# lifuguan/IGGT_official

Measured on NVIDIA H100. Metric: views/sec (518^2, V=8), higher is better.
Workload: dtype fp16

## Files before the change

### iggt_official_b200/csrc/gemm.cuh

```cuda
#pragma once
#include "ptx.cuh"
#include "launch.cuh"

namespace iggt {

enum GemmEpi : int {
  EPI_STORE16 = 0,
  EPI_RESID32 = 1,
  EPI_QKV = 2,
  EPI_STORE32 = 3,
  EPI_QKV_GATHER = 4,
};
__host__ __device__ constexpr bool epi_is_qkv(int e) { return e == EPI_QKV || e == EPI_QKV_GATHER; }

struct GemmParams {
  int M, N, K;
  int num_m_tiles, num_n_tiles, num_k_blocks;
  const float* bias;
  const float* gamma;
  int act;
  int qk_norm;
  int C;
  const float* qn_w; const float* qn_b; const float* kn_w; const float* kn_b;
  const float* rope_cos; const float* rope_sin;
  const int* pos_yx;
  int T;
  const void* addend; int add_rows; int add_ld;
  int conv_taps;
  int conv_C;
  int H, W, NB;
  int tiles_x, tiles_y;
  const void* resid;
  const void* resid2;
  int act_post;
  int round_out16;
  const CUtensorMap* gather_maps;
  int n_gather;
  int gather_col0;
  int gather_rows;
  int stream_k;
};

constexpr int GEMM_BM = 128;
constexpr int GEMM_BK = 64;
constexpr int GEMM_THREADS = 384;
constexpr int CONV_TW = 16;
constexpr int CONV_TH = 8;

template <int BN>
struct GemmSmem {
  static constexpr int A_BYTES = GEMM_BM * GEMM_BK * 2;
  static constexpr int B_BYTES = BN * GEMM_BK * 2;
  static constexpr int STAGE_BYTES = A_BYTES + B_BYTES;
  static constexpr int STG_BYTES = 16384;
  static constexpr int ACC_LD = BN + 8;
  static constexpr int ACC_BYTES = GEMM_BM * ACC_LD * 4;
  static constexpr int STAGES = BN == 128 ? 3 : 6;
  static constexpr int VEC_BYTES = BN * 4 + (BN * 4 > 1024 ? BN * 4 : 1024);
  static constexpr int TOTAL = STAGES * STAGE_BYTES + ACC_BYTES + 2 * STG_BYTES + 256  + VEC_BYTES;
};

template <bool BF16>
__device__ __forceinline__ float cvt16_to_f32(uint16_t h) {
  if constexpr (BF16) return __uint_as_float(static_cast<uint32_t>(h) << 16);
  else return __half2float(__ushort_as_half(h));
}
template <bool BF16>
__device__ __forceinline__ float round16(float x) {
  if constexpr (BF16) return __bfloat162float(__float2bfloat16_rn(x));
  else return __half2float(__float2half_rn(x));
}

__device__ __forceinline__ float apply_act(float x, int act) {
  if (act == 1) return gelu_fast(x);
  if (act == 2) return relu_nan(x);
  if (act == 3) return x > 0.0f ? x : 0.01f * x;
  return x;
}

struct WorkIter {
  int pos, end, step, kb_per_tile, num_tiles;
  bool sk;
  __device__ WorkIter(const GemmParams& p, int worker, int workers) {
    kb_per_tile = p.num_k_blocks;
    num_tiles = p.num_m_tiles * p.num_n_tiles;
    sk = p.stream_k != 0;
    if (sk) {
      const long total = static_cast<long>(num_tiles) * kb_per_tile;
      const long per = (total + workers - 1) / workers;
      const long b = static_cast<long>(worker) * per;
      pos = static_cast<int>(b < total ? b : total);
      end = static_cast<int>(b + per < total ? b + per : total);
      step = 0;
    } else {
      pos = worker; end = num_tiles; step = workers;
    }
  }
  __device__ bool next(int& tile, int& kb0, int& kb1) {
    if (pos >= end) return false;
    if (sk) {
      tile = pos / kb_per_tile;
      kb0 = pos - tile * kb_per_tile;
      const int room = end - pos;
      kb1 = kb0 + room < kb_per_tile ? kb0 + room : kb_per_tile;
      pos += kb1 - kb0;
    } else {
      tile = pos; kb0 = 0; kb1 = kb_per_tile; pos += step;
    }
    return true;
  }
};

template <int BN, int EPI, bool BF16, bool CONV>
__global__ void __launch_bounds__(GEMM_THREADS, 1)
gemm_wgmma_kernel(const __grid_constant__ CUtensorMap tmA, const __grid_constant__ CUtensorMap tmB,
                  const __grid_constant__ CUtensorMap tmC, const GemmParams p) {
  using SM = GemmSmem<BN>;
  constexpr int STAGES = SM::STAGES;
  constexpr int G = 2;
  extern __shared__ __align__(1024) uint8_t smem[];
  if ((smem_u32(smem) & 1023u) != 0) __trap();
  uint8_t* smem_a = smem;
  uint8_t* smem_b = smem + STAGES * SM::A_BYTES;
  float* acc_tile = reinterpret_cast<float*>(smem + STAGES * SM::STAGE_BYTES);
  uint8_t* staging = smem + STAGES * SM::STAGE_BYTES + SM::ACC_BYTES;
  uint64_t* bars = reinterpret_cast<uint64_t*>(staging + 2 * SM::STG_BYTES);
  uint64_t* full_bar = bars;
  uint64_t* empty_bar = bars + STAGES;
  float* epi_vec = reinterpret_cast<float*>(reinterpret_cast<uint8_t*>(bars) + 256);

  const int warp = threadIdx.x >> 5;
  const int lane = threadIdx.x & 31;
  const int worker = static_cast<int>(blockIdx.x);
  const int workers = static_cast<int>(gridDim.x);

  if (warp == 0 && lane == 0) {
    tma_prefetch_desc(&tmA);
    tma_prefetch_desc(&tmB);
    tma_prefetch_desc(&tmC);
  }
  if (warp == 1 && lane == 0) {
    for (int i = 0; i < STAGES; ++i) {
      mbar_init(&full_bar[i], 1);
      mbar_init(&empty_bar[i], G);
    }
    fence_barrier_init();
  }
  __syncthreads();
  griddep_wait();
  griddep_launch();

  if (warp < 4) {
    if (warp == 0 && lane == 0) {
      int stage = 0;
      uint32_t phase = 0;
      WorkIter work(p, worker, workers);
      int tile, kb0, kb1;
      while (work.next(tile, kb0, kb1)) {
        const int mt = tile / p.num_n_tiles;
        const int nt = tile % p.num_n_tiles;
        int img = 0, y0 = 0, x0 = 0;
        if constexpr (CONV) {
          const int per_img = p.tiles_x * p.tiles_y;
          img = mt / per_img;
          const int r = mt % per_img;
          y0 = (r / p.tiles_x) * CONV_TH;
          x0 = (r % p.tiles_x) * CONV_TW;
        }
        for (int kb = kb0; kb < kb1; ++kb) {
          mbar_wait(&empty_bar[stage], phase ^ 1);
          int dy = 0, dx = 0, c0 = 0;
          if constexpr (CONV) {
            const int cblocks = p.conv_C / GEMM_BK;
            const int tap = kb / cblocks;
            c0 = (kb % cblocks) * GEMM_BK;
            if (p.conv_taps == 9) { dy = tap / 3 - 1; dx = tap % 3 - 1; }
          }
          mbar_expect_tx(&full_bar[stage], SM::STAGE_BYTES);
          if constexpr (CONV) tma_load_4d(smem_a + stage * SM::A_BYTES, &tmA, &full_bar[stage], c0, x0 + dx, y0 + dy, img);
          else tma_load_2d(smem_a + stage * SM::A_BYTES, &tmA, &full_bar[stage], kb * GEMM_BK, mt * GEMM_BM);
          tma_load_2d(smem_b + stage * SM::B_BYTES, &tmB, &full_bar[stage], kb * GEMM_BK, nt * BN);
          if (++stage == STAGES) { stage = 0; phase ^= 1; }
        }
      }
    }
  } else {
    const int grp = (warp - 4) >> 2;
    const int ew = (warp - 4) & 3;
    const int row = ew * 32 + lane;
    const bool leader = (ew == 0 && lane == 0);
    constexpr int NBUF = 2 / G;
    uint8_t* const stg_grp = staging + grp * NBUF * SM::STG_BYTES;
    const uint32_t bar_id = 1 + grp;
    const int gtid = ew * 32 + lane;
    float* const vb = epi_vec;
    float* const vg = vb + BN;
    float* const vn = vb + BN;
    if constexpr (epi_is_qkv(EPI)) {
      if (p.qk_norm) {
        for (int i = gtid; i < 64; i += 128) {
          vn[i] = p.qn_w[i]; vn[64 + i] = p.qn_b[i]; vn[128 + i] = p.kn_w[i]; vn[192 + i] = p.kn_b[i];
        }
      }
    }
    int stage = 0;
    uint32_t phase = 0;
    uint32_t store_count = 0;
    WorkIter work(p, worker, workers);
    int tile, kb0, kb1;
    while (work.next(tile, kb0, kb1)) {
      const int mt = tile / p.num_n_tiles;
      const int nt = tile % p.num_n_tiles;
      const int n0 = nt * BN;
      float acc[BN / 2];
#pragma unroll
      for (int i = 0; i < BN / 2; ++i) acc[i] = 0.f;
      int prev_stage = -1;
      for (int kb = kb0; kb < kb1; ++kb) {
        mbar_wait(&full_bar[stage], phase);
        const uint32_t a_addr = smem_u32(smem_a + stage * SM::A_BYTES) + grp * (64 * 128);
        const uint32_t b_addr = smem_u32(smem_b + stage * SM::B_BYTES);
        wgmma_fence();
#pragma unroll
        for (int k = 0; k < GEMM_BK / 16; ++k) {
          const uint64_t da = make_desc_sw128(a_addr + k * 32, 1024);
          const uint64_t db = make_desc_sw128(b_addr + k * 32, 1024);
          if constexpr (BN == 128) wgmma_m64n128k16_ss<BF16>(acc, da, db, (kb != kb0 || k != 0) ? 1u : 0u);
          else wgmma_m64n64k16_ss<BF16>(acc, da, db, (kb != kb0 || k != 0) ? 1u : 0u);
        }
        wgmma_commit();
        wgmma_wait<1>();
        if (prev_stage >= 0 && gtid == 0) mbar_arrive(&empty_bar[prev_stage]);
        prev_stage = stage;
        if (++stage == STAGES) { stage = 0; phase ^= 1; }
      }
      wgmma_wait<0>();
      reg_fence(acc);
      if (prev_stage >= 0 && gtid == 0) mbar_arrive(&empty_bar[prev_stage]);

      int img = 0, y0 = 0, x0 = 0;
      long grow;
      if constexpr (CONV) {
        const int per_img = p.tiles_x * p.tiles_y;
        img = mt / per_img;
        const int r = mt % per_img;
        y0 = (r / p.tiles_x) * CONV_TH;
        x0 = (r % p.tiles_x) * CONV_TW;
        const int yy = y0 + row / CONV_TW, xx = x0 + row % CONV_TW;
        grow = (yy < p.H && xx < p.W && img < p.NB) ? ((long)img * p.H + yy) * p.W + xx : -1;
      } else {
        grow = (long)mt * GEMM_BM + row;
        if (grow >= p.M) grow = -1;
      }
      named_bar_sync(3, 128 * G);
      {
        const int r0 = grp * 64 + ew * 16 + (lane >> 2);
        float* const d0 = acc_tile + r0 * SM::ACC_LD + 2 * (lane & 3);
#pragma unroll
        for (int j = 0; j < BN / 8; ++j) {
          *reinterpret_cast<float2*>(d0 + 8 * j) = make_float2(acc[4 * j], acc[4 * j + 1]);
          *reinterpret_cast<float2*>(d0 + 8 * SM::ACC_LD + 8 * j) = make_float2(acc[4 * j + 2], acc[4 * j + 3]);
        }
      }
      for (int i = grp * 128 + gtid; i < BN; i += 128 * G) {
        const int col = n0 + i;
        vb[i] = (p.bias && col < p.N && kb0 == 0) ? __ldg(p.bias + col) : 0.f;
        if constexpr (EPI == EPI_RESID32) vg[i] = (p.gamma && col < p.N) ? __ldg(p.gamma + col) : 1.f;
      }
      named_bar_sync(3, 128 * G);
      const float* const t_row = acc_tile + row * SM::ACC_LD;

      if constexpr (EPI == EPI_STORE16 || epi_is_qkv(EPI)) {
        const int nvalid = min(BN / 64, (p.N - n0 + 63) / 64);
#pragma unroll 1
        for (int c64 = grp; c64 < nvalid; c64 += G) {
          const int col0 = n0 + c64 * 64;
          uint8_t* stg = stg_grp + (store_count % NBUF) * SM::STG_BYTES;
          if (leader) tma_store_wait_read<NBUF - 1>();
          named_bar_sync(bar_id, 128);
          float v[64];
#pragma unroll
          for (int i = 0; i < 64; i += 4) {
            const float4 a = *reinterpret_cast<const float4*>(t_row + c64 * 64 + i);
            v[i] = a.x; v[i + 1] = a.y; v[i + 2] = a.z; v[i + 3] = a.w;
          }
          {
#pragma unroll
            for (int i = 0; i < 64; i += 4) {
              const float4 b = *reinterpret_cast<const float4*>(vb + c64 * 64 + i);
              const float2 lo = fadd2(make_float2(v[i], v[i + 1]), make_float2(b.x, b.y));
              const float2 hi = fadd2(make_float2(v[i + 2], v[i + 3]), make_float2(b.z, b.w));
              v[i] = lo.x; v[i + 1] = lo.y; v[i + 2] = hi.x; v[i + 3] = hi.y;
            }
          }
          if constexpr (epi_is_qkv(EPI)) {
            if (p.qk_norm && col0 < 2 * p.C) {
              const bool is_k = col0 >= p.C;
              const float* nw = vn + (is_k ? 128 : 0);
              const float* nb = nw + 64;
              float s = 0.f;
#pragma unroll
              for (int i = 0; i < 64; ++i) { v[i] = round16<BF16>(v[i]); s += v[i]; }
              const float mean = s * (1.0f / 64.0f);
              float q = 0.f;
#pragma unroll
              for (int i = 0; i < 64; ++i) { const float d = v[i] - mean; q += d * d; }
              const float rstd = rsqrtf(q * (1.0f / 64.0f) + 1e-5f);
#pragma unroll
              for (int i = 0; i < 64; ++i) v[i] = (v[i] - mean) * rstd * nw[i] + nb[i];
              const int t = (grow >= 0) ? static_cast<int>(grow % p.T) : 0;
              const int py = __ldg(p.pos_yx + 2 * t), px = __ldg(p.pos_yx + 2 * t + 1);
#pragma unroll
              for (int h = 0; h < 2; ++h) {
                const int ps = h == 0 ? py : px;
                const float* cs = p.rope_cos + ps * 16;
                const float* sn = p.rope_sin + ps * 16;
#pragma unroll
                for (int i = 0; i < 16; ++i) {
                  const float c = __ldg(cs + i), s_ = __ldg(sn + i);
                  const float a = v[h * 32 + i], b = v[h * 32 + 16 + i];
                  v[h * 32 + i] = a * c - b * s_;
                  v[h * 32 + 16 + i] = b * c + a * s_;
                }
              }
            }
          } else {
            if (p.act == 1) {
#pragma unroll
              for (int i = 0; i < 64; i += 2) {
                const float2 g = gelu_fast2(make_float2(round16<BF16>(v[i]), round16<BF16>(v[i + 1])));
                v[i] = g.x; v[i + 1] = g.y;
              }
            } else if (p.act == 5) {
#pragma unroll
              for (int i = 0; i < 64; i += 2) {
                const float2 g = gelu_erfc2(make_float2(round16<BF16>(v[i]), round16<BF16>(v[i + 1])));
                v[i] = g.x; v[i + 1] = g.y;
              }
            } else if (p.act) {
#pragma unroll
              for (int i = 0; i < 64; ++i) v[i] = apply_act(v[i], p.act);
            }
            if (p.addend && grow >= 0) {
              const uint16_t* ad = reinterpret_cast<const uint16_t*>(p.addend) +
                                   (grow % p.add_rows) * (long)p.add_ld + col0;
#pragma unroll
              for (int i = 0; i < 64; i += 8) {
                if (col0 + i < p.N) {
                  const uint4 u = __ldg(reinterpret_cast<const uint4*>(ad + i));
                  const uint32_t w[4] = {u.x, u.y, u.z, u.w};
#pragma unroll
                  for (int j = 0; j < 4; ++j) {
                    v[i + 2 * j] += cvt16_to_f32<BF16>(static_cast<uint16_t>(w[j] & 0xFFFF));
                    v[i + 2 * j + 1] += cvt16_to_f32<BF16>(static_cast<uint16_t>(w[j] >> 16));
                  }
                }
              }
            }
            if constexpr (CONV) {
#pragma unroll
              for (int rr = 0; rr < 2; ++rr) {
                const void* rp = rr == 0 ? p.resid : p.resid2;
                if (rp && grow >= 0) {
                  const uint16_t* ad = reinterpret_cast<const uint16_t*>(rp) + grow * (long)p.N + col0;
#pragma unroll
                  for (int i = 0; i < 64; i += 8) {
                    if (col0 + i < p.N) {
                      const uint4 u = __ldg(reinterpret_cast<const uint4*>(ad + i));
                      const uint32_t w[4] = {u.x, u.y, u.z, u.w};
#pragma unroll
                      for (int j = 0; j < 4; ++j) {
                        v[i + 2 * j] += cvt16_to_f32<BF16>(static_cast<uint16_t>(w[j] & 0xFFFF));
                        v[i + 2 * j + 1] += cvt16_to_f32<BF16>(static_cast<uint16_t>(w[j] >> 16));
                      }
                    }
                  }
                }
              }
              if (p.act_post) {
#pragma unroll
                for (int i = 0; i < 64; ++i) v[i] = apply_act(v[i], p.act_post);
              }
            }
          }
          bool later_scene = false;
          if constexpr (EPI == EPI_QKV_GATHER) {
            if (p.n_gather > 0 && col0 >= p.gather_col0 && grow >= 0)
              later_scene = grow / p.gather_rows != (static_cast<long>(mt) * GEMM_BM) / p.gather_rows;
          }
#pragma unroll
          for (int c = 0; c < 8; ++c) {
            uint4 u;
            u.x = pack16x2<BF16>(v[c * 8 + 0], v[c * 8 + 1]);
            u.y = pack16x2<BF16>(v[c * 8 + 2], v[c * 8 + 3]);
            u.z = pack16x2<BF16>(v[c * 8 + 4], v[c * 8 + 5]);
            u.w = pack16x2<BF16>(v[c * 8 + 6], v[c * 8 + 7]);
            *reinterpret_cast<uint4*>(stg + row * 128 + ((c ^ (row & 7)) << 4)) = u;
            if constexpr (EPI == EPI_QKV_GATHER) {
              if (later_scene) {
                void* const* ptrs = reinterpret_cast<void* const*>(p.gather_maps + p.n_gather);
                const long* lds = reinterpret_cast<const long*>(ptrs + p.n_gather);
                const long scene = grow / p.gather_rows, rr = grow - scene * p.gather_rows;
                const long off = scene * __ldg(lds + 1) + rr * __ldg(lds) + (col0 - p.gather_col0) + c * 8;
                for (int r = 0; r < p.n_gather; ++r)
                  *reinterpret_cast<uint4*>(reinterpret_cast<uint16_t*>(ptrs[r]) + off) = u;
              }
            }
          }
          if constexpr (EPI == EPI_QKV_GATHER) {
            if (later_scene) __threadfence_system();
          }
          fence_proxy_async_smem();
          named_bar_sync(bar_id, 128);
          if (leader) {
            if constexpr (CONV) tma_store_4d(&tmC, stg, col0, x0, y0, img);
            else tma_store_2d(&tmC, stg, col0, mt * GEMM_BM);
            if constexpr (EPI == EPI_QKV_GATHER) {
              if (p.n_gather > 0 && col0 >= p.gather_col0) {
                const int row0 = mt * GEMM_BM, scene = row0 / p.gather_rows, r0 = row0 - scene * p.gather_rows;
                for (int r = 0; r < p.n_gather; ++r)
                  tma_store_3d(&p.gather_maps[r], stg, col0 - p.gather_col0, r0, scene);
              }
            }
            tma_store_commit();
          }
          ++store_count;
        }
      } else {
        const int nvalid = min(BN / 32, (p.N - n0 + 31) / 32);
#pragma unroll 1
        for (int c32 = grp; c32 < nvalid; c32 += G) {
          const int col0 = n0 + c32 * 32;
          uint8_t* stg = stg_grp + (store_count % NBUF) * SM::STG_BYTES;
          if (leader) tma_store_wait_read<NBUF - 1>();
          named_bar_sync(bar_id, 128);
          float v[32];
#pragma unroll
          for (int i = 0; i < 32; i += 4) {
            const float4 a = *reinterpret_cast<const float4*>(t_row + c32 * 32 + i);
            v[i] = a.x; v[i + 1] = a.y; v[i + 2] = a.z; v[i + 3] = a.w;
          }
#pragma unroll
          for (int i = 0; i < 32; i += 4) {
            const float4 b = *reinterpret_cast<const float4*>(vb + c32 * 32 + i);
            float2 lo = fadd2(make_float2(v[i], v[i + 1]), make_float2(b.x, b.y));
            float2 hi = fadd2(make_float2(v[i + 2], v[i + 3]), make_float2(b.z, b.w));
            if constexpr (EPI == EPI_RESID32) {
              if (p.round_out16 && !p.stream_k) {
                lo.x = round16<BF16>(lo.x); lo.y = round16<BF16>(lo.y);
                hi.x = round16<BF16>(hi.x); hi.y = round16<BF16>(hi.y);
              }
              const float4 g = *reinterpret_cast<const float4*>(vg + c32 * 32 + i);
              lo = fmul2(lo, make_float2(g.x, g.y));
              hi = fmul2(hi, make_float2(g.z, g.w));
            }
            v[i] = lo.x; v[i + 1] = lo.y; v[i + 2] = hi.x; v[i + 3] = hi.y;
          }
          if constexpr (EPI == EPI_STORE32) {
            if (p.act) {
#pragma unroll
              for (int i = 0; i < 32; ++i) v[i] = apply_act(v[i], p.act);
            }
          }
#pragma unroll
          for (int c = 0; c < 8; ++c) {
            float4 u = make_float4(v[c * 4], v[c * 4 + 1], v[c * 4 + 2], v[c * 4 + 3]);
            *reinterpret_cast<float4*>(stg + row * 128 + ((c ^ (row & 7)) << 4)) = u;
          }
          fence_proxy_async_smem();
          named_bar_sync(bar_id, 128);
          if (leader) {
            if constexpr (EPI == EPI_RESID32) tma_reduce_add_2d(&tmC, stg, col0, mt * GEMM_BM);
            else tma_store_2d(&tmC, stg, col0, mt * GEMM_BM);
            tma_store_commit();
          }
          ++store_count;
        }
      }
    }
    if (leader) {
      tma_store_wait_all<0>();
      if constexpr (EPI == EPI_QKV_GATHER) {
        if (p.n_gather > 0) __threadfence_system();
      }
    }
  }
}

}
```

### iggt_official_b200/csrc/ptx.cuh

```cuda
#pragma once
#include <cuda.h>
#include <cuda_fp16.h>
#include <cuda_bf16.h>
#include <cuda_runtime.h>
#include <stdint.h>

namespace iggt {

__device__ __forceinline__ uint32_t smem_u32(const void* p) {
  return static_cast<uint32_t>(__cvta_generic_to_shared(p));
}
__device__ __forceinline__ uint32_t lane_id() { return threadIdx.x & 31; }

__device__ __forceinline__ bool elect_one() {
  uint32_t pred = 0;
  asm volatile(
      "{\n\t.reg .pred P;\n\t"
      "elect.sync _|P, 0xffffffff;\n\t"
      "selp.b32 %0, 1, 0, P;\n\t}\n"
      : "=r"(pred));
  return pred != 0;
}

__device__ __forceinline__ void mbar_init(uint64_t* bar, uint32_t count) {
  asm volatile("mbarrier.init.shared::cta.b64 [%0], %1;" ::"r"(smem_u32(bar)), "r"(count));
}
__device__ __forceinline__ void fence_barrier_init() {
  asm volatile("fence.mbarrier_init.release.cluster;" ::: "memory");
}
__device__ __forceinline__ void mbar_expect_tx(uint64_t* bar, uint32_t bytes) {
  asm volatile("mbarrier.arrive.expect_tx.shared::cta.b64 _, [%0], %1;" ::"r"(smem_u32(bar)),
               "r"(bytes)
               : "memory");
}
__device__ __forceinline__ void mbar_arrive(uint64_t* bar) {
  asm volatile("mbarrier.arrive.shared::cta.b64 _, [%0];" ::"r"(smem_u32(bar)) : "memory");
}
__device__ __forceinline__ bool mbar_try_wait(uint64_t* bar, uint32_t parity) {
  uint32_t ok;
  asm volatile(
      "{\n\t.reg .pred P;\n\t"
      "mbarrier.try_wait.parity.shared::cta.b64 P, [%1], %2;\n\t"
      "selp.b32 %0, 1, 0, P;\n\t}\n"
      : "=r"(ok)
      : "r"(smem_u32(bar)), "r"(parity)
      : "memory");
  return ok != 0;
}
__device__ __forceinline__ void mbar_wait(uint64_t* bar, uint32_t parity) {
  while (!mbar_try_wait(bar, parity)) {
  }
}

__device__ __forceinline__ void fence_proxy_async_smem() {
  asm volatile("fence.proxy.async.shared::cta;" ::: "memory");
}
__device__ __forceinline__ void named_bar_sync(uint32_t id, uint32_t nthreads) {
  asm volatile("bar.sync %0, %1;" ::"r"(id), "r"(nthreads) : "memory");
}

__device__ __forceinline__ void tma_prefetch_desc(const CUtensorMap* m) {
  asm volatile("prefetch.tensormap [%0];" ::"l"(reinterpret_cast<uint64_t>(m)) : "memory");
}
__device__ __forceinline__ void tma_load_2d(void* smem, const CUtensorMap* m, uint64_t* bar,
                                            int32_t c0, int32_t c1) {
  asm volatile(
      "cp.async.bulk.tensor.2d.shared::cluster.global.mbarrier::complete_tx::bytes"
      " [%0], [%1, {%3, %4}], [%2];" ::"r"(smem_u32(smem)),
      "l"(reinterpret_cast<uint64_t>(m)), "r"(smem_u32(bar)), "r"(c0), "r"(c1)
      : "memory");
}
__device__ __forceinline__ void tma_load_3d(void* smem, const CUtensorMap* m, uint64_t* bar,
                                            int32_t c0, int32_t c1, int32_t c2) {
  asm volatile(
      "cp.async.bulk.tensor.3d.shared::cluster.global.mbarrier::complete_tx::bytes"
      " [%0], [%1, {%3, %4, %5}], [%2];" ::"r"(smem_u32(smem)),
      "l"(reinterpret_cast<uint64_t>(m)), "r"(smem_u32(bar)), "r"(c0), "r"(c1), "r"(c2)
      : "memory");
}
__device__ __forceinline__ void tma_load_4d(void* smem, const CUtensorMap* m, uint64_t* bar,
                                            int32_t c0, int32_t c1, int32_t c2, int32_t c3) {
  asm volatile(
      "cp.async.bulk.tensor.4d.shared::cluster.global.mbarrier::complete_tx::bytes"
      " [%0], [%1, {%3, %4, %5, %6}], [%2];" ::"r"(smem_u32(smem)),
      "l"(reinterpret_cast<uint64_t>(m)), "r"(smem_u32(bar)), "r"(c0), "r"(c1), "r"(c2), "r"(c3)
      : "memory");
}
__device__ __forceinline__ void tma_bulk_load_1d(void* smem, const void* gptr, uint32_t bytes, uint64_t* bar) {
  asm volatile("cp.async.bulk.shared::cluster.global.mbarrier::complete_tx::bytes [%0], [%1], %2, [%3];" ::"r"(
                   smem_u32(smem)),
               "l"(reinterpret_cast<uint64_t>(gptr)), "r"(bytes), "r"(smem_u32(bar))
               : "memory");
}
__device__ __forceinline__ void tma_store_2d(const CUtensorMap* m, const void* smem, int32_t c0,
                                             int32_t c1) {
  asm volatile("cp.async.bulk.tensor.2d.global.shared::cta.bulk_group [%0, {%2, %3}], [%1];" ::"l"(
                   reinterpret_cast<uint64_t>(m)),
               "r"(smem_u32(smem)), "r"(c0), "r"(c1)
               : "memory");
}
__device__ __forceinline__ void tma_store_3d(const CUtensorMap* m, const void* smem, int32_t c0, int32_t c1, int32_t c2) {
  asm volatile("cp.async.bulk.tensor.3d.global.shared::cta.bulk_group [%0, {%2, %3, %4}], [%1];" ::"l"(
                   reinterpret_cast<uint64_t>(m)),
               "r"(smem_u32(smem)), "r"(c0), "r"(c1), "r"(c2)
               : "memory");
}
__device__ __forceinline__ void tma_store_4d(const CUtensorMap* m, const void* smem, int32_t c0,
                                             int32_t c1, int32_t c2, int32_t c3) {
  asm volatile(
      "cp.async.bulk.tensor.4d.global.shared::cta.bulk_group [%0, {%2, %3, %4, %5}], [%1];" ::"l"(
          reinterpret_cast<uint64_t>(m)),
      "r"(smem_u32(smem)), "r"(c0), "r"(c1), "r"(c2), "r"(c3)
      : "memory");
}
__device__ __forceinline__ void tma_reduce_add_2d(const CUtensorMap* m, const void* smem,
                                                  int32_t c0, int32_t c1) {
  asm volatile(
      "cp.reduce.async.bulk.tensor.2d.global.shared::cta.add.tile.bulk_group [%0, {%2, %3}], [%1];" ::
          "l"(reinterpret_cast<uint64_t>(m)),
      "r"(smem_u32(smem)), "r"(c0), "r"(c1)
      : "memory");
}
__device__ __forceinline__ void tma_store_commit() {
  asm volatile("cp.async.bulk.commit_group;" ::: "memory");
}
template <int N>
__device__ __forceinline__ void tma_store_wait_read() {
  asm volatile("cp.async.bulk.wait_group.read %0;" ::"n"(N) : "memory");
}
template <int N>
__device__ __forceinline__ void tma_store_wait_all() {
  asm volatile("cp.async.bulk.wait_group %0;" ::"n"(N) : "memory");
}

__device__ __forceinline__ void wgmma_fence() { asm volatile("wgmma.fence.sync.aligned;" ::: "memory"); }
__device__ __forceinline__ void wgmma_commit() { asm volatile("wgmma.commit_group.sync.aligned;" ::: "memory"); }
template <int N>
__device__ __forceinline__ void wgmma_wait() {
  asm volatile("wgmma.wait_group.sync.aligned %0;" ::"n"(N) : "memory");
}
template <int R>
__device__ __forceinline__ void reg_fence(float (&d)[R]) {
#pragma unroll
  for (int i = 0; i < R; ++i) asm volatile("" : "+f"(d[i])::"memory");
}

#define IGGT_D8(o) "+f"(d[o]), "+f"(d[o + 1]), "+f"(d[o + 2]), "+f"(d[o + 3]), "+f"(d[o + 4]), "+f"(d[o + 5]), \
                   "+f"(d[o + 6]), "+f"(d[o + 7])
#define IGGT_WGMMA_SS_32(T)                                                                                     \
  asm volatile("{\n\t.reg .pred p;\n\tsetp.ne.b32 p, %18, 0;\n\t"                                               \
               "wgmma.mma_async.sync.aligned.m64n32k16.f32." T "." T " {%0, %1, %2, %3, %4, %5, %6, %7, %8, %9, %10, %11, %12, %13, %14, %15}, %16, %17, p, 1, 1, 0, 0;\n\t}\n" \
               : IGGT_D8(0), IGGT_D8(8)                                                                                          \
               : "l"(a_desc), "l"(b_desc), "r"(accumulate))
template <bool BF16>
__device__ __forceinline__ void wgmma_m64n32k16_ss(float (&d)[16], uint64_t a_desc, uint64_t b_desc, uint32_t accumulate) {
  if constexpr (BF16) IGGT_WGMMA_SS_32("bf16");
  else IGGT_WGMMA_SS_32("f16");
}
#define IGGT_WGMMA_SS_64(T)                                                                                     \
  asm volatile("{\n\t.reg .pred p;\n\tsetp.ne.b32 p, %34, 0;\n\t"                                               \
               "wgmma.mma_async.sync.aligned.m64n64k16.f32." T "." T " {%0, %1, %2, %3, %4, %5, %6, %7, %8, %9, %10, %11, %12, %13, %14, %15, %16, %17, %18, %19, %20, %21, %22, %23, %24, %25, %26, %27, %28, %29, %30, %31}, %32, %33, p, 1, 1, 0, 0;\n\t}\n" \
               : IGGT_D8(0), IGGT_D8(8), IGGT_D8(16), IGGT_D8(24)                                                                                          \
               : "l"(a_desc), "l"(b_desc), "r"(accumulate))
template <bool BF16>
__device__ __forceinline__ void wgmma_m64n64k16_ss(float (&d)[32], uint64_t a_desc, uint64_t b_desc, uint32_t accumulate) {
  if constexpr (BF16) IGGT_WGMMA_SS_64("bf16");
  else IGGT_WGMMA_SS_64("f16");
}
#define IGGT_WGMMA_SS_128(T)                                                                                     \
  asm volatile("{\n\t.reg .pred p;\n\tsetp.ne.b32 p, %66, 0;\n\t"                                               \
               "wgmma.mma_async.sync.aligned.m64n128k16.f32." T "." T " {%0, %1, %2, %3, %4, %5, %6, %7, %8, %9, %10, %11, %12, %13, %14, %15, %16, %17, %18, %19, %20, %21, %22, %23, %24, %25, %26, %27, %28, %29, %30, %31, %32, %33, %34, %35, %36, %37, %38, %39, %40, %41, %42, %43, %44, %45, %46, %47, %48, %49, %50, %51, %52, %53, %54, %55, %56, %57, %58, %59, %60, %61, %62, %63}, %64, %65, p, 1, 1, 0, 0;\n\t}\n" \
               : IGGT_D8(0), IGGT_D8(8), IGGT_D8(16), IGGT_D8(24), IGGT_D8(32), IGGT_D8(40), IGGT_D8(48), IGGT_D8(56)                                                                                          \
               : "l"(a_desc), "l"(b_desc), "r"(accumulate))
template <bool BF16>
__device__ __forceinline__ void wgmma_m64n128k16_ss(float (&d)[64], uint64_t a_desc, uint64_t b_desc, uint32_t accumulate) {
  if constexpr (BF16) IGGT_WGMMA_SS_128("bf16");
  else IGGT_WGMMA_SS_128("f16");
}
#define IGGT_WGMMA_RS_TB_64(T)                                                                                   \
  asm volatile("{\n\t.reg .pred p;\n\tsetp.ne.b32 p, %37, 0;\n\t"                                               \
               "wgmma.mma_async.sync.aligned.m64n64k16.f32." T "." T " {%0, %1, %2, %3, %4, %5, %6, %7, %8, %9, %10, %11, %12, %13, %14, %15, %16, %17, %18, %19, %20, %21, %22, %23, %24, %25, %26, %27, %28, %29, %30, %31}, {%32, %33, %34, %35}, %36, p, 1, 1, 1;\n\t}\n" \
               : IGGT_D8(0), IGGT_D8(8), IGGT_D8(16), IGGT_D8(24)                                                                                          \
               : "r"(a[0]), "r"(a[1]), "r"(a[2]), "r"(a[3]), "l"(b_desc), "r"(accumulate))
template <bool BF16>
__device__ __forceinline__ void wgmma_m64n64k16_rs_tb(float (&d)[32], const uint32_t (&a)[4], uint64_t b_desc,
                                                      uint32_t accumulate) {
  if constexpr (BF16) IGGT_WGMMA_RS_TB_64("bf16");
  else IGGT_WGMMA_RS_TB_64("f16");
}

__device__ __forceinline__ uint64_t make_desc_sw128(uint32_t smem_addr, uint32_t sbo_bytes) {
  uint64_t d = 0;
  d |= static_cast<uint64_t>((smem_addr & 0x3FFFF) >> 4);
  d |= static_cast<uint64_t>(1) << 16;
  d |= static_cast<uint64_t>((sbo_bytes >> 4) & 0x3FFF) << 32;
  d |= static_cast<uint64_t>(1) << 62;
  return d;
}

__device__ __forceinline__ uint32_t pack_f16x2(float a, float b) {
  __half2 h = __floats2half2_rn(a, b);
  return *reinterpret_cast<uint32_t*>(&h);
}
__device__ __forceinline__ uint32_t pack_bf16x2(float a, float b) {
  __nv_bfloat162 h = __floats2bfloat162_rn(a, b);
  return *reinterpret_cast<uint32_t*>(&h);
}
template <bool BF16>
__device__ __forceinline__ uint32_t pack16x2(float a, float b) {
  if constexpr (BF16) return pack_bf16x2(a, b);
  else return pack_f16x2(a, b);
}
__device__ __forceinline__ float relu_nan(float x) {
  float y;
  asm("max.NaN.f32 %0, %1, 0f00000000;" : "=f"(y) : "f"(x));
  return y;
}
__device__ __forceinline__ float gelu_erf(float x) {
  return 0.5f * x * (1.0f + erff(x * 0.70710678118654752440f));
}
__device__ __forceinline__ float ex2_approx(float x) {
  float y;
  asm("ex2.approx.ftz.f32 %0, %1;" : "=f"(y) : "f"(x));
  return y;
}
__device__ __forceinline__ float2 ffma2(float2 a, float2 b, float2 c) {
  return make_float2(__fmaf_rn(a.x, b.x, c.x), __fmaf_rn(a.y, b.y, c.y));
}
__device__ __forceinline__ float2 fadd2(float2 a, float2 b) {
  return make_float2(__fadd_rn(a.x, b.x), __fadd_rn(a.y, b.y));
}
__device__ __forceinline__ float2 fmul2(float2 a, float2 b) {
  return make_float2(__fmul_rn(a.x, b.x), __fmul_rn(a.y, b.y));
}
__device__ __forceinline__ float gelu_fast(float x) {
  const float z = fabsf(x) * 0.70710678118654752440f;
  const float t = __fdividef(1.0f, fmaf(0.3275911f, z, 1.0f));
  float poly = fmaf(t, 1.061405429f, -1.453152027f);
  poly = fmaf(poly, t, 1.421413741f);
  poly = fmaf(poly, t, -0.284496736f);
  poly = fmaf(poly, t, 0.254829592f);
  poly *= t;
  const float e = ex2_approx(-z * z * 1.4426950408889634f);
  const float erf_abs = fmaf(-poly, e, 1.0f);
  const float hx = 0.5f * x;
  return fmaf(hx, copysignf(erf_abs, x), hx);
}

__device__ __forceinline__ float2 gelu_fast2(float2 x) {
  const float2 ax = make_float2(fabsf(x.x), fabsf(x.y));
  const float2 z = fmul2(ax, make_float2(0.70710678118654752440f, 0.70710678118654752440f));
  const float2 den = ffma2(make_float2(0.3275911f, 0.3275911f), z, make_float2(1.0f, 1.0f));
  const float2 t = make_float2(__fdividef(1.0f, den.x), __fdividef(1.0f, den.y));
  float2 poly = ffma2(t, make_float2(1.061405429f, 1.061405429f), make_float2(-1.453152027f, -1.453152027f));
  poly = ffma2(poly, t, make_float2(1.421413741f, 1.421413741f));
  poly = ffma2(poly, t, make_float2(-0.284496736f, -0.284496736f));
  poly = ffma2(poly, t, make_float2(0.254829592f, 0.254829592f));
  poly = fmul2(poly, t);
  const float2 nz = make_float2(-z.x, -z.y);
  const float2 arg = fmul2(fmul2(nz, z), make_float2(1.4426950408889634f, 1.4426950408889634f));
  const float2 e = make_float2(ex2_approx(arg.x), ex2_approx(arg.y));
  const float2 erf_abs = ffma2(make_float2(-poly.x, -poly.y), e, make_float2(1.0f, 1.0f));
  const float2 hx = fmul2(make_float2(0.5f, 0.5f), x);
  return ffma2(hx, make_float2(copysignf(erf_abs.x, x.x), copysignf(erf_abs.y, x.y)), hx);
}


__device__ __forceinline__ float2 gelu_erfc2(float2 x) {
  const float2 hx = fmul2(x, make_float2(0.5f, 0.5f));
  const float2 na = make_float2(__uint_as_float(__float_as_uint(hx.x) | 0x80000000u),
                                __uint_as_float(__float_as_uint(hx.y) | 0x80000000u));
  float2 z = fmul2(na, make_float2(-1.4142135623730951f, -1.4142135623730951f));
  z.x = fminf(z.x, 4.3f);
  z.y = fminf(z.y, 4.3f);
  float2 q = ffma2(make_float2(-1.5555357094854116e-05f, -1.5555357094854116e-05f), z,
                   make_float2(0.0004183394485153258f, 0.0004183394485153258f));
  q = ffma2(q, z, make_float2(-0.0048510609194636345f, -0.0048510609194636345f));
  q = ffma2(q, z, make_float2(0.03291909396648407f, 0.03291909396648407f));
  q = ffma2(q, z, make_float2(-0.1511300802230835f, -0.1511300802230835f));
  q = ffma2(q, z, make_float2(-0.9178327322006226f, -0.9178327322006226f));
  q = ffma2(q, z, make_float2(-1.6279296875f, -1.6279296875f));
  const float2 pz = fmul2(q, z);
  const float2 e = make_float2(ex2_approx(pz.x), ex2_approx(pz.y));
  const float2 s = ffma2(na, make_float2(-1.0f, -1.0f), hx);
  return ffma2(na, e, s);
}

}
```

Baseline: 59.69.

## Ping-pong consumer warpgroups across tiles with register reallocation

Before, the two consumer warpgroups each took half of every 128-row tile. Now each warpgroup handles the whole 128-row tile (two m64 wgmma accumulators) and the two groups alternate tiles. Named barriers order the MMA phases and the epilogue phases, so one group's epilogue overlaps the other group's MMA. setmaxnreg moves registers from the producer warps to the consumers to hold the doubled accumulator. The cost is more register pressure, a shared accumulator tile and staging buffer that are now serialized, and more complex ring and phase bookkeeping.

```diff
diff --git a/iggt_official_b200/csrc/gemm.cuh b/iggt_official_b200/csrc/gemm.cuh
--- a/iggt_official_b200/csrc/gemm.cuh
+++ b/iggt_official_b200/csrc/gemm.cuh
@@ -117,7 +117,7 @@
                   const __grid_constant__ CUtensorMap tmC, const GemmParams p) {
   using SM = GemmSmem<BN>;
   constexpr int STAGES = SM::STAGES;
-  constexpr int G = 2;
+  constexpr uint32_t BAR_MMA_DONE = 3, BAR_EPI_DONE = 5;
   extern __shared__ __align__(1024) uint8_t smem[];
   if ((smem_u32(smem) & 1023u) != 0) __trap();
   uint8_t* smem_a = smem;
@@ -142,7 +142,7 @@
   if (warp == 1 && lane == 0) {
     for (int i = 0; i < STAGES; ++i) {
       mbar_init(&full_bar[i], 1);
-      mbar_init(&empty_bar[i], G);
+      mbar_init(&empty_bar[i], 1);
     }
     fence_barrier_init();
   }
@@ -151,6 +151,7 @@
   griddep_launch();
 
   if (warp < 4) {
+    reg_dealloc<40>();
     if (warp == 0 && lane == 0) {
       int stage = 0;
       uint32_t phase = 0;
@@ -185,48 +186,64 @@
       }
     }
   } else {
-    const int grp = (warp - 4) >> 2;
+    reg_alloc<232>();
+    const int wg = (warp - 4) >> 2;
     const int ew = (warp - 4) & 3;
     const int row = ew * 32 + lane;
     const bool leader = (ew == 0 && lane == 0);
-    constexpr int NBUF = 2 / G;
-    uint8_t* const stg_grp = staging + grp * NBUF * SM::STG_BYTES;
-    const uint32_t bar_id = 1 + grp;
+    constexpr int NBUF = 2;
+    const uint32_t bar_id = 1 + wg;
     const int gtid = ew * 32 + lane;
     float* const vb = epi_vec;
     float* const vg = vb + BN;
     float* const vn = vb + BN;
     if constexpr (epi_is_qkv(EPI)) {
-      if (p.qk_norm) {
+      if (p.qk_norm && wg == 0) {
         for (int i = gtid; i < 64; i += 128) {
           vn[i] = p.qn_w[i]; vn[64 + i] = p.qn_b[i]; vn[128 + i] = p.kn_w[i]; vn[192 + i] = p.kn_b[i];
         }
       }
     }
-    int stage = 0;
-    uint32_t phase = 0;
     uint32_t store_count = 0;
     WorkIter work(p, worker, workers);
-    int tile, kb0, kb1;
-    while (work.next(tile, kb0, kb1)) {
+    int tile, kb0, kb1, ntile, nkb0, nkb1;
+    bool more = work.next(ntile, nkb0, nkb1);
+    uint32_t ring = 0;
+    int seg_len = 0;
+    for (int seg = 0; more; ++seg) {
+      ring += seg_len;
+      tile = ntile; kb0 = nkb0; kb1 = nkb1;
+      seg_len = kb1 - kb0;
+      more = work.next(ntile, nkb0, nkb1);
+      if ((seg & 1) != wg) continue;
       const int mt = tile / p.num_n_tiles;
       const int nt = tile % p.num_n_tiles;
       const int n0 = nt * BN;
-      float acc[BN / 2];
-#pragma unroll
-      for (int i = 0; i < BN / 2; ++i) acc[i] = 0.f;
+      if (seg > 0) named_bar_sync(BAR_MMA_DONE + (wg ^ 1), 256);
+      int stage = static_cast<int>(ring % STAGES);
+      uint32_t phase = (ring / STAGES) & 1;
+      float acc[2][BN / 2];
+#pragma unroll
+      for (int h = 0; h < 2; ++h) {
+#pragma unroll
+        for (int i = 0; i < BN / 2; ++i) acc[h][i] = 0.f;
+      }
       int prev_stage = -1;
       for (int kb = kb0; kb < kb1; ++kb) {
         mbar_wait(&full_bar[stage], phase);
-        const uint32_t a_addr = smem_u32(smem_a + stage * SM::A_BYTES) + grp * (64 * 128);
+        const uint32_t a_addr = smem_u32(smem_a + stage * SM::A_BYTES);
         const uint32_t b_addr = smem_u32(smem_b + stage * SM::B_BYTES);
         wgmma_fence();
 #pragma unroll
         for (int k = 0; k < GEMM_BK / 16; ++k) {
-          const uint64_t da = make_desc_sw128(a_addr + k * 32, 1024);
           const uint64_t db = make_desc_sw128(b_addr + k * 32, 1024);
-          if constexpr (BN == 128) wgmma_m64n128k16_ss<BF16>(acc, da, db, (kb != kb0 || k != 0) ? 1u : 0u);
-          else wgmma_m64n64k16_ss<BF16>(acc, da, db, (kb != kb0 || k != 0) ? 1u : 0u);
+          const uint32_t accumulate = (kb != kb0 || k != 0) ? 1u : 0u;
+#pragma unroll
+          for (int h = 0; h < 2; ++h) {
+            const uint64_t da = make_desc_sw128(a_addr + h * (64 * 128) + k * 32, 1024);
+            if constexpr (BN == 128) wgmma_m64n128k16_ss<BF16>(acc[h], da, db, accumulate);
+            else wgmma_m64n64k16_ss<BF16>(acc[h], da, db, accumulate);
+          }
         }
         wgmma_commit();
         wgmma_wait<1>();
@@ -234,8 +251,10 @@
         prev_stage = stage;
         if (++stage == STAGES) { stage = 0; phase ^= 1; }
       }
+      if (more) named_bar_arrive(BAR_MMA_DONE + wg, 256);
       wgmma_wait<0>();
-      reg_fence(acc);
+      reg_fence(acc[0]);
+      reg_fence(acc[1]);
       if (prev_stage >= 0 && gtid == 0) mbar_arrive(&empty_bar[prev_stage]);
 
       int img = 0, y0 = 0, x0 = 0;
@@ -252,30 +271,31 @@
         grow = (long)mt * GEMM_BM + row;
         if (grow >= p.M) grow = -1;
       }
-      named_bar_sync(3, 128 * G);
-      {
-        const int r0 = grp * 64 + ew * 16 + (lane >> 2);
+      if (seg > 0) named_bar_sync(BAR_EPI_DONE + (wg ^ 1), 256);
+#pragma unroll
+      for (int h = 0; h < 2; ++h) {
+        const int r0 = h * 64 + ew * 16 + (lane >> 2);
         float* const d0 = acc_tile + r0 * SM::ACC_LD + 2 * (lane & 3);
 #pragma unroll
         for (int j = 0; j < BN / 8; ++j) {
-          *reinterpret_cast<float2*>(d0 + 8 * j) = make_float2(acc[4 * j], acc[4 * j + 1]);
-          *reinterpret_cast<float2*>(d0 + 8 * SM::ACC_LD + 8 * j) = make_float2(acc[4 * j + 2], acc[4 * j + 3]);
-        }
-      }
-      for (int i = grp * 128 + gtid; i < BN; i += 128 * G) {
+          *reinterpret_cast<float2*>(d0 + 8 * j) = make_float2(acc[h][4 * j], acc[h][4 * j + 1]);
+          *reinterpret_cast<float2*>(d0 + 8 * SM::ACC_LD + 8 * j) = make_float2(acc[h][4 * j + 2], acc[h][4 * j + 3]);
+        }
+      }
+      for (int i = gtid; i < BN; i += 128) {
         const int col = n0 + i;
         vb[i] = (p.bias && col < p.N && kb0 == 0) ? __ldg(p.bias + col) : 0.f;
         if constexpr (EPI == EPI_RESID32) vg[i] = (p.gamma && col < p.N) ? __ldg(p.gamma + col) : 1.f;
       }
-      named_bar_sync(3, 128 * G);
+      named_bar_sync(bar_id, 128);
       const float* const t_row = acc_tile + row * SM::ACC_LD;
 
       if constexpr (EPI == EPI_STORE16 || epi_is_qkv(EPI)) {
         const int nvalid = min(BN / 64, (p.N - n0 + 63) / 64);
 #pragma unroll 1
-        for (int c64 = grp; c64 < nvalid; c64 += G) {
+        for (int c64 = 0; c64 < nvalid; ++c64) {
           const int col0 = n0 + c64 * 64;
-          uint8_t* stg = stg_grp + (store_count % NBUF) * SM::STG_BYTES;
+          uint8_t* stg = staging + (store_count % NBUF) * SM::STG_BYTES;
           if (leader) tma_store_wait_read<NBUF - 1>();
           named_bar_sync(bar_id, 128);
           float v[64];
@@ -429,9 +449,9 @@
       } else {
         const int nvalid = min(BN / 32, (p.N - n0 + 31) / 32);
 #pragma unroll 1
-        for (int c32 = grp; c32 < nvalid; c32 += G) {
+        for (int c32 = 0; c32 < nvalid; ++c32) {
           const int col0 = n0 + c32 * 32;
-          uint8_t* stg = stg_grp + (store_count % NBUF) * SM::STG_BYTES;
+          uint8_t* stg = staging + (store_count % NBUF) * SM::STG_BYTES;
           if (leader) tma_store_wait_read<NBUF - 1>();
           named_bar_sync(bar_id, 128);
           float v[32];
@@ -477,6 +497,8 @@
           ++store_count;
         }
       }
+      if (leader) tma_store_wait_read<0>();
+      if (more) named_bar_arrive(BAR_EPI_DONE + wg, 256);
     }
     if (leader) {
       tma_store_wait_all<0>();
diff --git a/iggt_official_b200/csrc/ptx.cuh b/iggt_official_b200/csrc/ptx.cuh
--- a/iggt_official_b200/csrc/ptx.cuh
+++ b/iggt_official_b200/csrc/ptx.cuh
@@ -57,6 +57,18 @@
 }
 __device__ __forceinline__ void named_bar_sync(uint32_t id, uint32_t nthreads) {
   asm volatile("bar.sync %0, %1;" ::"r"(id), "r"(nthreads) : "memory");
+}
+__device__ __forceinline__ void named_bar_arrive(uint32_t id, uint32_t nthreads) {
+  asm volatile("bar.arrive %0, %1;" ::"r"(id), "r"(nthreads) : "memory");
+}
+
+template <uint32_t N>
+__device__ __forceinline__ void reg_dealloc() {
+  asm volatile("setmaxnreg.dec.sync.aligned.u32 %0;" ::"n"(N));
+}
+template <uint32_t N>
+__device__ __forceinline__ void reg_alloc() {
+  asm volatile("setmaxnreg.inc.sync.aligned.u32 %0;" ::"n"(N));
 }
 
 __device__ __forceinline__ void tma_prefetch_desc(const CUtensorMap* m) {
```

Result: faster. 63.09 (median of 6 runs) (+5.7%).
